# facebookresearch/lightplane

Hardware: AMD Instinct MI355X
Metric: Mrays/sec fwd+bwd, 64^3x16ch triplane @128 samples; peak bwd mem (MB) (higher is better)
Workload: dtype f32

## Files before the change

### lightplane_amd/csrc/lp_mfma_common.h

```cpp
#pragma once
#include <stdlib.h>

#include "lp_device.h"
#include "lp_splat_walk.h"
#include "lp_host.h"
#include "lp_plane_range.h"

namespace lp {

typedef float f32x16 __attribute__((ext_vector_type(16)));

LP_DEV constexpr int featq(int q, int h) { return (q & 3) + 8 * (q >> 2) + 4 * h; }

#define LP_MFMA(a, b, c) __builtin_amdgcn_mfma_f32_32x32x2f32((a), (b), (c), 0, 0, 0)

LP_DEV int opaque_zero() {
  int z = 0;
  asm volatile("" : "+s"(z));
  return z;
}

constexpr int HID = 32;
constexpr int W_LD = 33;
constexpr int WAVES = 4;
// ... 18 lines not shown
};

struct Lds {
  static constexpr int WT1 = 0;
  static constexpr int WT2 = WT1 + 32 * W_LD;
  static constexpr int WO1 = WT2 + 32 * W_LD;
  static constexpr int WC1 = WO1 + 32 * W_LD;
  static constexpr int BIAS = WC1 + 32 * W_LD;
  static constexpr int WO2 = BIAS + 4 * 32;
  static constexpr int WC2 = WO2 + 32;
  static constexpr int HB = WC2 + 32 * 4;
  static constexpr int INF = HB + 8;
  static constexpr int FWD_END = INF + MAX_INF;
};

LP_DEV f32x16 load_bias(const float* lds, int which, int h, int zo) {
  const float4* b = reinterpret_cast<const float4*>(lds + Lds::BIAS + which * 32 + 4 * h + zo);
  f32x16 acc;
#pragma unroll
  for (int j = 0; j < 4; ++j) {
    const float4 v = b[2 * j];
    acc[4 * j + 0] = v.x; acc[4 * j + 1] = v.y; acc[4 * j + 2] = v.z; acc[4 * j + 3] = v.w;
  }
  return acc;
}

LP_DEV int wave_min_i(int v) {
#pragma unroll
  for (int m = 32; m >= 1; m >>= 1) { const int o = __shfl_xor(v, m); v = o < v ? o : v; }
  return __builtin_amdgcn_readfirstlane(v);
}
struct WaveRanges {
  unsigned lo3, hi3;
  static constexpr unsigned G = 0x20080200u;
  LP_DEV unsigned mask(int s) const {
    s = __builtin_amdgcn_readfirstlane(s);
    const unsigned sss = (unsigned)(s < 511 ? s : 511) * 0x00100401u;
    return ((sss | G) - lo3) & ((hi3 | G) - sss) & G;
  }
  static constexpr unsigned bit(int g) { return 0x200u << (10 * g); }
};
constexpr int RANGE_MAX_S = 511;
LP_DEV WaveRanges wave_ranges_full() { return WaveRanges{0u, 0x1ff7fdffu}; }
template <int GM>
LP_DEV WaveRanges wave_plane_ranges(const LpRendererArgs& a, const Ray& ray, bool valid, bool plain) {
  WaveRanges w = wave_ranges_full();
  if (GM == GM_GENERIC) return w;
  const int S = a.march.num_samples;
  if (!plain || S > RANGE_MAX_S || __ballot(!valid) != 0) return w;
  const LpGrid* g = a.grid.grids;
  const int W = g[0].W, H = g[0].H, D = (GM == GM_TRIPLANE) ? g[1].D : g[0].D;
  const AxisSpans ax = ray_axis_spans(ray.ox, ray.oy, ray.oz, ray.dx, ray.dy, ray.dz, ray.near_t, ray.far_t, S, W, H, D);
#pragma unroll
  for (int p = 0; p < (GM == GM_TRIPLANE ? 3 : 1); ++p) {
    const SampleSpan sp = (GM == GM_TRIPLANE) ? plane_span(ax, p, S) : voxel_span(ax, S);
    const int lo = wave_min_i(sp.lo), hi = -wave_min_i(-sp.hi);
    if (p == 0) w.lo3 = w.hi3 = 0u;
    w.lo3 |= (unsigned)(hi < lo ? 511 : lo) << (10 * p);
    w.hi3 |= (unsigned)(hi < lo ? 0 : hi) << (10 * p);
  }
  if (GM == GM_VOXEL) {
    w.lo3 *= 0x00100401u;
    w.hi3 *= 0x00100401u;
  }
  w.lo3 = (unsigned)__builtin_amdgcn_readfirstlane((int)w.lo3);
  w.hi3 = (unsigned)__builtin_amdgcn_readfirstlane((int)w.hi3);
  return w;
}

template <int C>
LP_DEV void gather_tap(const float* data, int row, float w, int h, float (&x0)[C / 2]) {
  const float4* src = reinterpret_cast<const float4*>(data + (int64_t)(row < 0 ? 0 : row) * C + 4 * h);
#pragma unroll
  for (int j = 0; j < C / 8; ++j) {
    const float4 v = src[2 * j];
    x0[4 * j + 0] = fmaf(w, v.x, x0[4 * j + 0]);
    x0[4 * j + 1] = fmaf(w, v.y, x0[4 * j + 1]);
    x0[4 * j + 2] = fmaf(w, v.z, x0[4 * j + 2]);
    x0[4 * j + 3] = fmaf(w, v.w, x0[4 * j + 3]);
  }
}

template <int C>
LP_DEV void gather_taps4(const float* data, const int* row, const float* w, float keep, int h, float (&x0)[C / 2]) {
  float4 v[4][C / 8];
#pragma unroll
  for (int k = 0; k < 4; ++k) {
    const float4* src = reinterpret_cast<const float4*>(data + (int64_t)(row[k] < 0 ? 0 : row[k]) * C + 4 * h);
#pragma unroll
    for (int j = 0; j < C / 8; ++j) v[k][j] = src[2 * j];
  }
  __builtin_amdgcn_sched_barrier(0);
#pragma unroll
  for (int k = 0; k < 4; ++k) {
    const float wk = w[k] * keep;
#pragma unroll
    for (int j = 0; j < C / 8; ++j) {
      x0[4 * j + 0] = fmaf(wk, v[k][j].x, x0[4 * j + 0]);
      x0[4 * j + 1] = fmaf(wk, v[k][j].y, x0[4 * j + 1]);
      x0[4 * j + 2] = fmaf(wk, v[k][j].z, x0[4 * j + 2]);
// ... 498 lines not shown
```

### lightplane_amd/csrc/lp_plane_range.h

```cpp
#pragma once
#include <math.h>

#if defined(__HIPCC__)
#define LP_HD __host__ __device__ inline
#else
#define LP_HD inline
#endif

namespace lp {

struct SampleSpan {
  int lo, hi;
};

LP_HD SampleSpan span_full(int S) { return SampleSpan{0, S - 1}; }
LP_HD SampleSpan span_none(int S) { return SampleSpan{S, -1}; }
LP_HD SampleSpan span_meet(SampleSpan a, SampleSpan b, int S) {
  const SampleSpan m{a.lo > b.lo ? a.lo : b.lo, a.hi < b.hi ? a.hi : b.hi};
  return m.lo > m.hi ? span_none(S) : m;
}
LP_HD SampleSpan span_hull(SampleSpan a, SampleSpan b) {
  return SampleSpan{a.lo < b.lo ? a.lo : b.lo, a.hi > b.hi ? a.hi : b.hi};
}

LP_HD SampleSpan axis_sample_span(float o, float d, float near_t, float far_t, int S, int size) {
  if (S < 2) return span_full(S);
  const float L = 1.0f + 1.0f / (float)size;
  const float per = (float)(S - 1) / (far_t - near_t);
  const float inv = 1.0f / d;
  float s0 = ((-L - o) * inv - near_t) * per;
  float s1 = ((L - o) * inv - near_t) * per;
  if (s0 > s1) { const float t = s0; s0 = s1; s1 = t; }
  const float err = 1.9073486e-6f * fabsf(per) * ((L + fabsf(o)) * fabsf(inv) + fabsf(near_t) + fabsf(far_t));
  if (!(err < 0.5f)) return span_full(S);
  if (!(s0 <= (float)S && s1 >= -1.0f)) return span_none(S);
  const int lo = (int)floorf(fmaxf(s0, 0.0f)) - 1;
  const int hi = (int)ceilf(fminf(s1, (float)(S - 1))) + 1;
  return SampleSpan{lo < 0 ? 0 : lo, hi > S - 1 ? S - 1 : hi};
}

struct AxisSpans {
  SampleSpan x, y, z;
};
LP_HD AxisSpans ray_axis_spans(float ox, float oy, float oz, float dx, float dy, float dz, float near_t, float far_t, int S, int W,
                               int H, int D) {
  return AxisSpans{axis_sample_span(ox, dx, near_t, far_t, S, W), axis_sample_span(oy, dy, near_t, far_t, S, H),
                   axis_sample_span(oz, dz, near_t, far_t, S, D)};
}
LP_HD SampleSpan plane_span(const AxisSpans& a, int g, int S) {
  return g == 0 ? span_meet(a.x, a.y, S) : (g == 1 ? span_meet(a.x, a.z, S) : span_meet(a.y, a.z, S));
}
LP_HD SampleSpan voxel_span(const AxisSpans& a, int S) { return span_meet(span_meet(a.x, a.y, S), a.z, S); }

}
```

### lightplane_amd/csrc/lp_renderer_mfma.hip

```cpp
#include "lp_mfma_common.h"
#include "lp_bf3.h"

namespace lp {

template <int C, int GM, int OCC, int NC, bool SEGF = false>
__global__ void __launch_bounds__(256, OCC) renderer_fwd_bf3(const LpRendererArgs a, const MfmaParams mp) {
  extern __shared__ __attribute__((aligned(16))) float lds[];
  stage_weights_bf3<C>(a, mp, lds, false, 256);
  __syncthreads();
  const float* sm = lds - Lds::BIAS;
  const char* fimg = reinterpret_cast<const char*>(lds) + LdsBf3<C>::FWD_IMG;
  const int lane = threadIdx.x & 63, wave = threadIdx.x >> 6;
  const int h = lane >> 5, r = lane & 31;
  const int seg_len = LP_SEG_LEN * mp.seg_blocks;
  const int n_seg = SEGF ? (a.march.num_samples + seg_len - 1) / seg_len : 1;
  const int blk = SEGF ? (int)blockIdx.x / n_seg : (int)blockIdx.x;
  const int seg = SEGF ? (int)blockIdx.x - blk * n_seg : 0;
  const int64_t ray_id = ((int64_t)blk * WAVES + wave) * RAYS_PER_WAVE + r;
  const bool valid = ray_id < a.rays.n_rays;
  const int64_t rid = valid ? ray_id : 0;
  const Ray ray = load_ray(a.rays, rid);
  float cb[16];
  {
    float enc[16];
    load_encoding(a, rid, h, enc);
    color_prebias_bf3<C>(sm, fimg, lane, enc, cb);
  }
  const int s_tot = a.march.num_samples + a.march.num_samples_inf;
  const int n_ckpt = ckpt_count(a.march);
  const float delta0 = (a.march.num_samples > 1) ? (ray.far_t - ray.near_t) / (float)(a.march.num_samples - 1) : 1.0f;
  float nlt = 0.0f, nlt_lo = 0.0f, t_prev = 1.0f, len = 0.0f, depth_prev = 0.0f;
  int s_last = s_tot - 1;
  float facc[4] = {0.0f, 0.0f, 0.0f, 0.0f};
  Sample<C> nx;
  Act<C> t;
  const int s_lo = SEGF ? seg * seg_len : 0;
  const int s_hi = SEGF ? ((s_lo + seg_len < s_tot) ? s_lo + seg_len : s_tot) : s_tot;
  const bool plain_march = !SEGF && a.march.num_samples_inf == 0 && !a.march.contract_coords && !a.scaffold && !(a.noise_sigma > 0.0f);
  const WaveRanges rg = wave_plane_ranges<GM>(a, ray, valid, plain_march);
  if (SEGF && s_lo > 0) {
    sample_geometry<C>(a, sm, ray, s_lo - 1, nx);
    depth_prev = nx.depth;
  }
  for (int s = s_lo; s < s_hi; ++s) {
    fetch_sample<C, GM, true>(a, sm, ray, s, h, nx, rg.mask(s));
    const float depth = nx.depth, occ = nx.occ;
#pragma unroll
    for (int q = 0; q < C / 2; ++q) t.x0[q] = nx.x0[q];
    const int zo = opaque_zero();
    const Heads hd = decode_bf3<C, NC>(sm, fimg, lane, cb, t, zo);
    const float delta = (s == 0) ? delta0 : depth - depth_prev;
    depth_prev = depth;
    float raw = hd.raw_o;
    if (a.noise_sigma > 0.0f) raw = raw + sample_noise(rid, s, a.rays.n_rays, s_tot, a.noise_seed) * a.noise_sigma;
    const float opacity = a.gain * softplus_f(raw) * occ;
    nlt_add(nlt, nlt_lo, opacity * delta);
    if (!SEGF && a.neg_log_t_ckpt && valid && h == 0) {
      const int ck = ckpt_index(s, a.march);
      if (ck >= 0) *reinterpret_cast<float2*>(a.neg_log_t_ckpt + (ray_id * n_ckpt + ck) * 2) = make_float2(nlt, nlt_lo);
    }
    const float tr = __expf(-nlt);
    const float w = t_prev - tr;
    t_prev = tr;
    len = fmaf(w, depth, len);
#pragma unroll
    for (int c = 0; c < NC; ++c) facc[c] = fmaf(w, sigmoid_f(hd.raw_c[c]) * occ, facc[c]);
    if (a.seg_prefix && valid && h == 0 && (((s + 1) % LP_SEG_LEN) == 0 || s == a.march.num_samples - 1)) {
      float4* dst = reinterpret_cast<float4*>(a.seg_prefix + (ray_id * segment_count(a.march) + s / LP_SEG_LEN) * 8);
      dst[0] = make_float4(len, facc[0], facc[1], facc[2]);
      dst[1] = make_float4(NC == 4 ? facc[3] : 0.0f, nlt, nlt_lo, 0.0f);
    }
    if (a.stop_neg_log_t > 0.0f && __ballot(valid && nlt < a.stop_neg_log_t) == 0) {
      s_last = s;
      break;
    }
  }
  if (!SEGF && valid && h == 0) {
    write_ray_outputs(a, ray_id, len, nlt, facc);
    if (a.neg_log_t_ckpt)
      *reinterpret_cast<float2*>(a.neg_log_t_ckpt + (ray_id * n_ckpt + n_ckpt - 1) * 2) = make_float2((float)s_last, nlt_lo);
  }
}

// ... 300 lines not shown
```

### lightplane_amd/csrc/lp_renderer_mfma_bwd.h

```cpp
#pragma once
#include "lp_mfma_common.h"
#include <type_traits>

#include "lp_bf3.h"

namespace lp {

#ifdef LP_ASM_MARKS
#define LP_MARK(n) asm volatile("; LPMARK " n)
#else
#define LP_MARK(n)
#endif
typedef float f32x4 __attribute__((ext_vector_type(4)));
#define LP_MFMA16(a, b, c) __builtin_amdgcn_mfma_f32_16x16x4f32((a), (b), (c), 0, 0, 0)

constexpr int T_LD = 36;

LP_DEV constexpr int pi16(int m) { return m < 4 ? 2 * m : (m < 12 ? 2 * (m - 4) + 1 : 2 * (m - 8)); }

LP_DEV void lds_barrier() { asm volatile("s_waitcnt lgkmcnt(0)\n\ts_barrier" ::: "memory"); }

LP_DEV void tile_store_fm(float* tile, int r, int h, const float (&v)[16]) {
#pragma unroll
  for (int q = 0; q < 16; ++q) tile[featq(q, h) * T_LD + r] = v[q];
// ... 34 lines not shown
  const u32x2_t ua = __builtin_bit_cast(u32x2_t, a), ub = __builtin_bit_cast(u32x2_t, b);
  return (u32x4_t){ua.x, ua.y, ub.x, ub.y};
}
template <int STRIDE_BYTES>
LP_DEV f32x4 dw_quadrant_bf(const char* wave0b, int x_off, int y_off, int v0, int v1, f32x4 acc, f32x4& acc_db, unsigned onehot, bool do_db = true) {
  const u32x4_t oh = {onehot, onehot, onehot, onehot};
#pragma unroll 1
  for (int v = v0; v < v1; ++v) {
    const char* base = wave0b + v * STRIDE_BYTES;
    const u32x4_t b2 = limb_tile_operand(base + y_off + LT_LIMB);
    const u32x4_t a1 = limb_tile_operand(base + x_off);
    if (do_db) acc_db = LP_MFMA16B(oh, b2, acc_db);
    acc = LP_MFMA16B(a1, b2, acc);
    const u32x4_t b1 = limb_tile_operand(base + y_off);
    if (do_db) acc_db = LP_MFMA16B(oh, b1, acc_db);
    acc = LP_MFMA16B(a1, b1, acc);
    const u32x4_t a2 = limb_tile_operand(base + x_off + LT_LIMB);
    acc = LP_MFMA16B(a2, b1, acc);
  }
  return acc;
}

struct LdsB3 {
  static constexpr int XT = 0;
  static constexpr int YT = 32 * T_LD;
  static constexpr int TS = 2 * 32 * T_LD;
  static constexpr int PER_WAVE = TS + 5 * 32;
};
template <int C, int NW>
struct Bf3Lds {
  static constexpr int IMG_END = (NW == 8) ? LdsBf3<C>::BWD_END : LdsBf3Rm<C>::END;
  static constexpr int CB = IMG_END + NW * LdsB3::PER_WAVE * 4;
  static constexpr bool CB_LDS = (NW == 8) ? (C == 16) : (CB + NW * 64 * 16 * 4) * 2 <= 160 * 1024;
  static constexpr int TOTAL = CB + (CB_LDS ? NW * 64 * 16 * 4 : 0);
};

template <int C, int GM, bool PLAIN, int NC, int NW, bool SEG = false, bool DUMP = false, bool F32 = false>
__global__ void __launch_bounds__(64 * NW, NW == 8 ? 1 : 2) renderer_bwd_bf3(const LpRendererArgs a, const MfmaParams mp) {
  constexpr int DXL = F32 ? 3 : 2;
  constexpr bool DWB = !F32;
  using M = Lds;
  using L = LdsBf3<C>;
  using R = LdsBf3Rm<C>;
  using B = LdsB3;
  constexpr int WAVES3 = NW;
  extern __shared__ __attribute__((aligned(16))) float lds[];
  if (NW == 8) stage_weights_bf3<C>(a, mp, lds, true, 64 * NW);
  else stage_weights_rm<C>(a, mp, lds, 64 * NW);
  const float* const sm = lds - M::BIAS;
  const char* const fimg = reinterpret_cast<const char*>(lds) + L::FWD_IMG;
  const char* const bimg = reinterpret_cast<const char*>(lds) + L::BWD_IMG;
  const char* const rimg = reinterpret_cast<const char*>(lds);
  const int lane = threadIdx.x & 63;
  const int wave = __builtin_amdgcn_readfirstlane((int)(threadIdx.x >> 6));
  const int h = lane >> 5, r = lane & 31;
  float* const wave0 = reinterpret_cast<float*>(reinterpret_cast<char*>(lds) + Bf3Lds<C, NW>::IMG_END);
  float* const wv = wave0 + wave * B::PER_WAVE;
  float* const xt = wv + B::XT;
  float* const yt = wv + B::YT;
  float* const ts = wv + B::TS;

  constexpr bool seg_on = SEG;
  const int n_rec = seg_on ? segment_count(a.march) : 1;
  const int seg_len = LP_SEG_LEN * mp.seg_blocks;
  const int n_seg = seg_on ? (a.march.num_samples + seg_len - 1) / seg_len : 1;
  const int blk = seg_on ? (int)blockIdx.x / n_seg : (int)blockIdx.x;
  const int seg = seg_on ? (int)blockIdx.x - blk * n_seg : 0;
// ... 63 lines not shown
  auto rho = [](int k) { return (k & 0x15) | ((k & 2) << 2) | ((k & 8) >> 2); };
  char* const xrow = reinterpret_cast<char*>(wv) + B::XT * 4 + rm_off(rho(r), 4 * h);
  char* const yrow = xrow + (B::YT - B::XT) * 4;
  const int xq_off = B::XT * 4 + rm_off(rho(8 * ka + (m16 >> 2)), 4 * (m16 & 3)) + 32 * mi;
  const int yq_off = B::YT * 4 + rm_off(rho(8 * ka + (m16 >> 2)), 4 * (m16 & 3)) + 32 * ni;
  f32x4 dq_b = {0, 0, 0, 0};
  auto onehot = [&](int li) -> unsigned { return (lane & 15) == li ? 0x3F803F80u : 0u; };
  const int a_off_t1 = (C == 16) ? B::XT + pi16(m16) * T_LD + 8 * ka : a_off;
  const int t1_v0 = (C == 16) ? 2 * (wave >> 1) : v0, t1_v1 = (C == 16) ? 2 * (wave >> 1) + 2 : v0 + 4;
  f32x4 dq_t1 = {0, 0, 0, 0}, dq_t2 = {0, 0, 0, 0}, dq_o1 = {0, 0, 0, 0}, dq_c1 = {0, 0, 0, 0};
  float db_t1 = 0.0f, db_t2 = 0.0f, db_o1 = 0.0f, db_c1 = 0.0f;
  float dwo2 = 0.0f, dwc2[4] = {0.0f, 0.0f, 0.0f, 0.0f};
  float dbo2 = 0.0f, dbc2[4] = {0.0f, 0.0f, 0.0f, 0.0f};
  const bool gg = a.grad_grid_list[0] != nullptr;

  float nlt = a.neg_log_t[rid];
  float suffix = 0.0f, p_next = 0.0f;
  if (seg_on) {
    const float4* pj = reinterpret_cast<const float4*>(a.seg_prefix + (rid * n_rec + s_begin / LP_SEG_LEN) * 8);
    const float4* pt = reinterpret_cast<const float4*>(a.seg_prefix + (rid * n_rec + n_rec - 1) * 8);
    const float4 j0 = pj[0], j1 = pj[1], t0 = pt[0];
    nlt = j1.y;
    nlt_lo = j1.z;
    if (seg < n_seg - 1) {
      float rest = g_len * (t0.x - j0.x);
      rest = fmaf(gfeat[0], t0.y - j0.y, rest);
      rest = fmaf(gfeat[1], t0.z - j0.z, rest);
      rest = fmaf(gfeat[2], t0.w - j0.w, rest);
      if (NC == 4) rest = fmaf(gfeat[3], pt[1].x - j1.x, rest);
      suffix = -rest;
    }
  }
  const WaveRanges rg = wave_plane_ranges<GM>(a, ray, valid, PLAIN && !SEG);
  Sample<C> nx;
  fetch_sample<C, GM, false, PLAIN>(a, sm, ray, s_begin, h, nx);
  for (int s = s_begin; s >= s_lo; --s) {
    const bool on = PLAIN || s <= s_last_w;
    const unsigned pm = rg.mask(s);
    const bool ggs = gg && pm != 0u;
    const float depth = nx.depth, occ = nx.occ, x = nx.x, y = nx.y, z = nx.z;
    float x0[C / 2];
#pragma unroll
    for (int q = 0; q < C / 2; ++q) x0[q] = nx.x0[q];
    const int zo = opaque_zero();
    const float* ldz = sm + zo;
    auto Af = [&](auto layer) {
      constexpr int l = decltype(layer)::value;
      if constexpr (NW == 8) return ASlots{fimg + zo, l == 0 ? L::CH_T1 : l == 1 ? L::CH_T2 : l == 2 ? L::CH_O1 : L::CH_C1};
      else return AColsFwd{rimg + zo + (l == 0 ? R::L_T1 : l == 1 ? R::L_T2 : l == 2 ? R::L_O1 : R::L_C1), l == 0 ? R::ST_T1 : R::ST_32};
    };
    auto Ab = [&](auto layer) {
      constexpr int l = decltype(layer)::value;
      if constexpr (NW == 8) return ASlots{bimg + zo, l == 0 ? L::CB_T1 : l == 1 ? L::CB_T2 : l == 2 ? L::CB_O1 : L::CB_C1};
      else return ARowsBwd{rimg + zo + (l == 0 ? R::L_T1 : l == 1 ? R::L_T2 : l == 2 ? R::L_O1 : R::L_C1), l == 0 ? R::ST_T1 : R::ST_32,
                           l == 0 ? C - 1 : 31};
    };
    using I0 = std::integral_constant<int, 0>; using I1 = std::integral_constant<int, 1>;
    using I2 = std::integral_constant<int, 2>; using I3 = std::integral_constant<int, 3>;

    LP_MARK("fwd");
    float h1[16];
    float e[16];
    unsigned ho_mask = 0, hc_mask = 0;
    Heads hd;
    {
      f32x16 acc;
      {
        acc = layer_bf3v<C / 16>(Af(I0{}), lane, x0, load_bias(sm, 0, h, zo));
#pragma unroll
        for (int q = 0; q < 16; ++q) h1[q] = relu_f(acc[q]);
      }
      acc = layer_bf3v<2>(Af(I1{}), lane, h1, load_bias(sm, 1, h, zo));
#pragma unroll
      for (int q = 0; q < 16; ++q) {
        e[q] = relu_f(acc[q]);
      }
      float ho[16], hc[16];
      {
        f32x16 acc_o = load_bias(sm, 2, h, zo), acc_c;
        if (CBL) {
#pragma unroll
          for (int i = 0; i < 4; ++i) {
            const float4 v = *reinterpret_cast<const float4*>(cbt + zo + ((i + cb_rot) & 3) * 4);
            acc_c[4 * i] = v.x; acc_c[4 * i + 1] = v.y; acc_c[4 * i + 2] = v.z; acc_c[4 * i + 3] = v.w;
          }
        } else {
#pragma unroll
          for (int q = 0; q < 16; ++q) acc_c[q] = cb[q];
        }
        layer2_bf3v<2>(Af(I2{}), Af(I3{}), lane, e, acc_o, acc_c);
#pragma unroll
        for (int q = 0; q < 16; ++q) {
          ho[q] = relu_f(acc_o[q]);
          hc[q] = relu_f(acc_c[q]);
        }
      }
      hd = heads_forward<NC>(sm, h, ho, hc, zo);
#pragma unroll
      for (int q = 0; q < 16; ++q) {
        ho_mask = mask_bit(ho_mask, ho[q], q);
        hc_mask = mask_bit(hc_mask, hc[q], q);
      }
      if constexpr (DUMP) {
        unsigned m1 = 0, m2 = 0, mo = 0, mc = 0;
#pragma unroll
        for (int q = 0; q < 16; ++q) {
          const unsigned bit = 1u << featq(q, h);
          m1 |= (h1[q] > 0.0f) ? bit : 0u;
          m2 |= (e[q] > 0.0f) ? bit : 0u;
          mo |= ((ho_mask >> q) & 1u) ? bit : 0u;
          mc |= ((hc_mask >> q) & 1u) ? bit : 0u;
        }
        m1 |= __shfl_xor(m1, 32); m2 |= __shfl_xor(m2, 32); mo |= __shfl_xor(mo, 32); mc |= __shfl_xor(mc, 32);
        if (valid && h == 0) {
          uint32_t* d = mp.relu_dump + (rid * s_tot + s) * 5;
          d[0] = m1; d[1] = m2; d[2] = mo; d[3] = mc; d[4] = on ? 1u : 2u;
        }
      }
      LP_SCHED_FENCE();
      if (want_params) {
        tile_store_fm(xt, r, h, ho);
        tile_store_fm(yt, r, h, hc);
      }
      LP_SCHED_FENCE();
    }

    LP_MARK("compositing");
    const float depth_prev =
        PLAIN ? ray.near_t + lin01((s > 0) ? s - 1 : 0, a.march.num_samples) * (ray.far_t - ray.near_t)
              : sample_depth_tab((s > 0) ? s - 1 : 0, a.march, ray.near_t, ray.far_t, sm + M::INF);
    const float delta = (s == 0) ? delta0 : depth - depth_prev;
    float raw = hd.raw_o;
    if (!PLAIN && a.noise_sigma > 0.0f)
      raw = raw + sample_noise(rid, s, a.rays.n_rays, s_tot, a.noise_seed) * a.noise_sigma;
    const float opacity = a.gain * softplus_f(raw) * occ;
    if (on && a.neg_log_t_ckpt) {
      const int ck = PLAIN ? ((((s + 1) % LP_NLT_CKPT) == 0 || s == s_tot - 1) ? s / LP_NLT_CKPT : -1)
                           : ckpt_index(s, a.march);
      if (ck >= 0) {
        const float2 c2 = *reinterpret_cast<const float2*>(a.neg_log_t_ckpt + (rid * n_ckpt + ck) * 2);
        nlt = c2.x;
        nlt_lo = c2.y;
      }
    }
    const float t_i = __expf(-nlt);
    nlt_add(nlt, nlt_lo, on ? -(opacity * delta) : 0.0f);
    if (!(nlt > 0.0f)) { nlt = 0.0f; nlt_lo = 0.0f; }
    const float t_im1 = __expf(-nlt);
    const float w = t_im1 - t_i;
    float sg[4];
    float p_i = g_len * depth;
#pragma unroll
    for (int c = 0; c < 4; ++c) {
      sg[c] = (c < NC) ? sigmoid_f(hd.raw_c[c]) : 0.0f;
      if (c < NC) p_i = fmaf(gfeat[c], sg[c] * occ, p_i);
    }
    suffix = on ? fmaf(t_i, p_i - p_next, suffix) : suffix;
    p_next = on ? p_i : p_next;
    const float d_a = suffix + g_nlt;
    const bool contrib = valid && on;
    const float dro = contrib ? d_a * delta * a.gain * occ * d_softplus_f(raw) : 0.0f;
    float drc[4];
#pragma unroll
    for (int c = 0; c < 4; ++c) drc[c] = (c < NC && contrib) ? w * gfeat[c] * occ * sg[c] * (1.0f - sg[c]) : 0.0f;

    LP_MARK("heads_bwd");
    float dhc[16];
    {
      const float* wc2 = sm + M::WC2 + 16 * h + opaque_zero();
#pragma unroll
      for (int j = 0; j < 4; ++j) {
#pragma unroll
        for (int i = 0; i < 4; ++i) {
          const int q = 4 * j + i;
          const float4 wc = *reinterpret_cast<const float4*>(wc2 + (8 * j + i) * 4);
          float v = drc[0] * wc.x;
          v = fmaf(drc[1], wc.y, v);
          v = fmaf(drc[2], wc.z, v);
          if (NC > 3) v = fmaf(drc[3], wc.w, v);
          dhc[q] = mask_apply(hc_mask, q, v);
        }
        LP_SCHED_FENCE();
      }
    }
    if (h == 0) {
      dbo2 += dro;
#pragma unroll
      for (int c = 0; c < NC; ++c) dbc2[c] += drc[c];
    }
    if (want_params) {
      if (h == 0) {
        ts[r] = dro;
#pragma unroll
        for (int c = 0; c < NC; ++c) ts[(1 + c) * 32 + r] = drc[c];
      }
      const float* xf = xt + r * T_LD + 16 * h;
      const float* yf = yt + r * T_LD + 16 * h;
      const float* tf = ts + 16 * h;
#pragma unroll
      for (int i = 0; i < 4; ++i) {
        const float4 hov = *reinterpret_cast<const float4*>(xf + 4 * i);
        const float4 hcv = *reinterpret_cast<const float4*>(yf + 4 * i);
        const float4 d0 = *reinterpret_cast<const float4*>(tf + 4 * i);
        dwo2 = fmaf(hov.x, d0.x, dwo2); dwo2 = fmaf(hov.y, d0.y, dwo2);
        dwo2 = fmaf(hov.z, d0.z, dwo2); dwo2 = fmaf(hov.w, d0.w, dwo2);
#pragma unroll
        for (int c = 0; c < NC; ++c) {
          const float4 dc = *reinterpret_cast<const float4*>(tf + (1 + c) * 32 + 4 * i);
          dwc2[c] = fmaf(hcv.x, dc.x, dwc2[c]); dwc2[c] = fmaf(hcv.y, dc.y, dwc2[c]);
          dwc2[c] = fmaf(hcv.z, dc.z, dwc2[c]); dwc2[c] = fmaf(hcv.w, dc.w, dwc2[c]);
        }
        LP_SCHED_FENCE();
      }
    }
    LP_SCHED_FENCE();

    LP_MARK("c1");
#ifndef LP_NO_PRIO
    __builtin_amdgcn_s_setprio(1);
#endif
    f32x16 acc = (f32x16){0};
    {
      if constexpr (DWB) {
        if (want_params) limb_tile_store<2>(xrow, e);
        acc = layer_dxv<2, DXL>(Ab(I3{}), lane, dhc, acc, want_params ? yrow : nullptr);
      } else {
        if (want_params) {
          tile_store_fm(xt, r, h, e);
          tile_store_fm(yt, r, h, dhc);
        }
        acc = layer_dxv<2, DXL>(Ab(I3{}), lane, dhc, acc);
      }
#pragma unroll
      for (int q = 0; q < 16; ++q) dsum[q] += dhc[q];
      if (want_params) {
        lds_barrier();
        if constexpr (DWB) dq_c1 = dw_quadrant_bf<B::PER_WAVE * 4>(reinterpret_cast<const char*>(wave0), xq_off, yq_off, v0, v0 + 4, dq_c1, dq_b, onehot(0));
        else dq_c1 = dw_quadrant<B::PER_WAVE>(wave0, a_off, b_off, v0, v0 + 4, dq_c1, db_c1);
        lds_barrier();
      }
    }
    LP_SCHED_FENCE();
    LP_MARK("o1");
    {
      float dho[16];
#pragma unroll
      for (int j = 0; j < 4; ++j) {
        const float4 wo = *reinterpret_cast<const float4*>(ldz + M::WO2 + 8 * j + 4 * h);
        dho[4 * j + 0] = mask_apply(ho_mask, 4 * j + 0, dro * wo.x);
        dho[4 * j + 1] = mask_apply(ho_mask, 4 * j + 1, dro * wo.y);
        dho[4 * j + 2] = mask_apply(ho_mask, 4 * j + 2, dro * wo.z);
        dho[4 * j + 3] = mask_apply(ho_mask, 4 * j + 3, dro * wo.w);
      }
      if constexpr (DWB) {
        acc = layer_dxv<2, DXL>(Ab(I2{}), lane, dho, acc, want_params ? yrow : nullptr);
      } else {
        if (want_params) tile_store_fm(yt, r, h, dho);
        acc = layer_dxv<2, DXL>(Ab(I2{}), lane, dho, acc);
      }
      if (want_params) {
        lds_barrier();
        if constexpr (DWB) dq_o1 = dw_quadrant_bf<B::PER_WAVE * 4>(reinterpret_cast<const char*>(wave0), xq_off, yq_off, v0, v0 + 4, dq_o1, dq_b, onehot(1));
        else dq_o1 = dw_quadrant<B::PER_WAVE>(wave0, a_off, b_off, v0, v0 + 4, dq_o1, db_o1);
        lds_barrier();
      }
    }
    float de[16];
#pragma unroll
    for (int q = 0; q < 16; ++q) de[q] = (e[q] > 0.0f) ? acc[q] : 0.0f;
    LP_SCHED_FENCE();
    LP_MARK("t2");
    float dh1[16];
    {
      if constexpr (DWB) {
        if (want_params) limb_tile_store<2>(xrow, h1);
        acc = layer_dxv<2, DXL>(Ab(I1{}), lane, de, (f32x16){0}, want_params ? yrow : nullptr);
      } else {
        if (want_params) {
          tile_store_fm(xt, r, h, h1);
          tile_store_fm(yt, r, h, de);
        }
        acc = layer_dxv<2, DXL>(Ab(I1{}), lane, de, (f32x16){0});
      }
      if (want_params) {
        lds_barrier();
        if constexpr (DWB) dq_t2 = dw_quadrant_bf<B::PER_WAVE * 4>(reinterpret_cast<const char*>(wave0), xq_off, yq_off, v0, v0 + 4, dq_t2, dq_b, onehot(2));
        else dq_t2 = dw_quadrant<B::PER_WAVE>(wave0, a_off, b_off, v0, v0 + 4, dq_t2, db_t2);
      }
#pragma unroll
      for (int q = 0; q < 16; ++q) dh1[q] = (h1[q] > 0.0f) ? acc[q] : 0.0f;
      if (want_params) lds_barrier();
    }
    LP_SCHED_FENCE();
    LP_MARK("t1");
    {
      if constexpr (DWB) {
        if (want_params) limb_tile_store<C / 16>(xrow, x0);
        if (ggs) {
          acc = layer_dxv<2, DXL>(Ab(I0{}), lane, dh1, (f32x16){0}, want_params ? yrow : nullptr);
        } else if (want_params) {
          limb_tile_store<2>(yrow, dh1);
        }
      } else {
        if (want_params) {
#pragma unroll
          for (int q = 0; q < C / 2; ++q) xt[featq(q, h) * T_LD + r] = x0[q];
          tile_store_fm(yt, r, h, dh1);
        }
        if (ggs) {
          acc = layer_dxv<2, DXL>(Ab(I0{}), lane, dh1, (f32x16){0});
        }
      }
      if (want_params) {
        lds_barrier();
        if constexpr (DWB) dq_t1 = dw_quadrant_bf<B::PER_WAVE * 4>(reinterpret_cast<const char*>(wave0), (C == 16) ? xq_off - 32 * mi : xq_off, yq_off, t1_v0, t1_v1, dq_t1, dq_b, onehot(3));
        else dq_t1 = dw_quadrant<B::PER_WAVE>(wave0, a_off_t1, b_off, t1_v0, t1_v1, dq_t1, db_t1);
        lds_barrier();
      }
    }
    if (ggs) {
#pragma unroll
      for (int q = 0; q < C / 2; ++q) xt[featq(q, h) * DX_LD + r] = acc[q];
    }
    LP_SCHED_FENCE();
    LP_MARK("fetch");
    __builtin_amdgcn_s_setprio(0);
    const bool live = valid && on && !(a.march.mask_out_of_bounds && !point_in_bounds(x, y, z));
    if (s > s_lo) fetch_sample<C, GM, true, PLAIN>(a, sm, ray, s - 1, h, nx, rg.mask(s - 1));
    LP_SCHED_FENCE();
    LP_MARK("scatter");
    if (ggs) {
      if constexpr (GM == GM_TRIPLANE) {
        scatter_triplane<C>(a.grad_grid_list, a.grid, ray.b, x, y, z, live, lane, xt, yt, pm);
      } else {
        const int ng = (GM == GM_VOXEL) ? 1 : a.grid.n_grids;
#pragma unroll 1
        for (int g = 0; g < ng; ++g)
          scatter_grid<C, GM>(a.grad_grid_list[g], a.grid.grids[g], ray.b, x, y, z, live, lane, xt, yt);
      }
    }
  }

  LP_MARK("epilogue");
  {
    f32x16 acc;
    if constexpr (NW == 8) acc = layer_bf3v<2>(ASlots{bimg, L::CB_C1}, lane, dsum, (f32x16){0});
    else acc = layer_bf3v<2>(ARowsBwd{rimg + R::L_C1, R::ST_32, 31}, lane, dsum, (f32x16){0});
    if (valid && a.grad_encoding && !seg_on) {
      float4* dst = reinterpret_cast<float4*>(a.grad_encoding + ray_id * HID + 4 * h);
#pragma unroll
      for (int j = 0; j < 4; ++j) dst[2 * j] = make_float4(acc[4 * j], acc[4 * j + 1], acc[4 * j + 2], acc[4 * j + 3]);
    } else if (valid && a.grad_encoding) {
      float* dst = a.grad_encoding + ray_id * HID + 4 * h;
#pragma unroll
      for (int j = 0; j < 4; ++j)
#pragma unroll
        for (int i = 0; i < 4; ++i) atomic_add_f32(dst + 8 * j + i, acc[4 * j + i]);
    }
  }
  if (want_params) {
    {
// ... 134 lines not shown
```

Measured before the change: 30.94.

## Skip MLP recompute and backprop for samples outside all planes via constant-feature shortcut

Samples where every plane mask is empty see zero features, so their MLP outputs are the same constant. The forward pass and backward pass now compute this zero-feature MLP once per wave or workgroup and reuse it for those samples. In the backward pass, gradients from skipped samples are accumulated and pushed through the MLP once in a single deferred extra iteration. This is meant to remove per-sample MLP work in empty regions, at the cost of extra LDS, a workgroup-wide range exchange with barriers, and more complex control flow.

Result: no change. 31.30 (median of 6 runs) (+1.1%).

```diff
diff --git a/lightplane_amd/csrc/lp_mfma_common.h b/lightplane_amd/csrc/lp_mfma_common.h
--- a/lightplane_amd/csrc/lp_mfma_common.h
+++ b/lightplane_amd/csrc/lp_mfma_common.h
@@ -74,16 +74,21 @@
 }
 struct WaveRanges {
   unsigned lo3, hi3;
-  static constexpr unsigned G = 0x20080200u;
+  static constexpr unsigned G = RANGE3_GUARD;
   LP_DEV unsigned mask(int s) const {
     s = __builtin_amdgcn_readfirstlane(s);
-    const unsigned sss = (unsigned)(s < 511 ? s : 511) * 0x00100401u;
-    return ((sss | G) - lo3) & ((hi3 | G) - sss) & G;
+    return range3_mask(lo3, hi3, s);
   }
   static constexpr unsigned bit(int g) { return 0x200u << (10 * g); }
+  LP_DEV bool any_empty(int s0, int s1) const {
+    if (lo3 == RANGE3_FULL_LO && hi3 == RANGE3_FULL_HI) return false;
+    bool any = false;
+    for (int s = s0; s <= s1; ++s) any = any || mask(s) == 0u;
+    return any;
+  }
 };
-constexpr int RANGE_MAX_S = 511;
-LP_DEV WaveRanges wave_ranges_full() { return WaveRanges{0u, 0x1ff7fdffu}; }
+constexpr int RANGE_MAX_S = RANGE3_MAX_S;
+LP_DEV WaveRanges wave_ranges_full() { return WaveRanges{RANGE3_FULL_LO, RANGE3_FULL_HI}; }
 template <int GM>
 LP_DEV WaveRanges wave_plane_ranges(const LpRendererArgs& a, const Ray& ray, bool valid, bool plain) {
   WaveRanges w = wave_ranges_full();
@@ -93,21 +98,34 @@
   const LpGrid* g = a.grid.grids;
   const int W = g[0].W, H = g[0].H, D = (GM == GM_TRIPLANE) ? g[1].D : g[0].D;
   const AxisSpans ax = ray_axis_spans(ray.ox, ray.oy, ray.oz, ray.dx, ray.dy, ray.dz, ray.near_t, ray.far_t, S, W, H, D);
+  w.lo3 = w.hi3 = 0u;
 #pragma unroll
   for (int p = 0; p < (GM == GM_TRIPLANE ? 3 : 1); ++p) {
     const SampleSpan sp = (GM == GM_TRIPLANE) ? plane_span(ax, p, S) : voxel_span(ax, S);
-    const int lo = wave_min_i(sp.lo), hi = -wave_min_i(-sp.hi);
-    if (p == 0) w.lo3 = w.hi3 = 0u;
-    w.lo3 |= (unsigned)(hi < lo ? 511 : lo) << (10 * p);
-    w.hi3 |= (unsigned)(hi < lo ? 0 : hi) << (10 * p);
+    range3_set(w.lo3, w.hi3, p, SampleSpan{wave_min_i(sp.lo), -wave_min_i(-sp.hi)});
   }
   if (GM == GM_VOXEL) {
-    w.lo3 *= 0x00100401u;
-    w.hi3 *= 0x00100401u;
+    w.lo3 *= RANGE3_ONES;
+    w.hi3 *= RANGE3_ONES;
   }
   w.lo3 = (unsigned)__builtin_amdgcn_readfirstlane((int)w.lo3);
   w.hi3 = (unsigned)__builtin_amdgcn_readfirstlane((int)w.hi3);
   return w;
+}
+template <int NW>
+LP_DEV WaveRanges workgroup_ranges(const WaveRanges& w, unsigned* xch, int wave, int lane) {
+  if (lane == 0) {
+    xch[2 * wave] = w.lo3;
+    xch[2 * wave + 1] = w.hi3;
+  }
+  __syncthreads();
+  WaveRanges g = w;
+#pragma unroll
+  for (int v = 0; v < NW; ++v) range3_hull(g.lo3, g.hi3, xch[2 * v], xch[2 * v + 1]);
+  __syncthreads();
+  g.lo3 = (unsigned)__builtin_amdgcn_readfirstlane((int)g.lo3);
+  g.hi3 = (unsigned)__builtin_amdgcn_readfirstlane((int)g.hi3);
+  return g;
 }
 
 template <int C>
diff --git a/lightplane_amd/csrc/lp_plane_range.h b/lightplane_amd/csrc/lp_plane_range.h
--- a/lightplane_amd/csrc/lp_plane_range.h
+++ b/lightplane_amd/csrc/lp_plane_range.h
@@ -52,4 +52,28 @@
 }
 LP_HD SampleSpan voxel_span(const AxisSpans& a, int S) { return span_meet(span_meet(a.x, a.y, S), a.z, S); }
 
+constexpr int RANGE3_MAX_S = 511;
+constexpr unsigned RANGE3_GUARD = 0x20080200u;
+constexpr unsigned RANGE3_ONES = 0x00100401u;
+constexpr unsigned RANGE3_FULL_LO = 0u, RANGE3_FULL_HI = 0x1ff7fdffu;
+LP_HD void range3_set(unsigned& lo3, unsigned& hi3, int p, SampleSpan sp) {
+  lo3 |= (unsigned)(sp.hi < sp.lo ? 511 : sp.lo) << (10 * p);
+  hi3 |= (unsigned)(sp.hi < sp.lo ? 0 : sp.hi) << (10 * p);
 }
+LP_HD unsigned range3_mask(unsigned lo3, unsigned hi3, int s) {
+  const unsigned sss = (unsigned)(s < 511 ? s : 511) * RANGE3_ONES;
+  return ((sss | RANGE3_GUARD) - lo3) & ((hi3 | RANGE3_GUARD) - sss) & RANGE3_GUARD;
+}
+LP_HD void range3_hull(unsigned& lo3, unsigned& hi3, unsigned l, unsigned h) {
+  unsigned lo = 0u, hi = 0u;
+  for (int p = 0; p < 3; ++p) {
+    const unsigned a = (lo3 >> (10 * p)) & 511u, b = (l >> (10 * p)) & 511u;
+    const unsigned c = (hi3 >> (10 * p)) & 511u, d = (h >> (10 * p)) & 511u;
+    lo |= (a < b ? a : b) << (10 * p);
+    hi |= (c > d ? c : d) << (10 * p);
+  }
+  lo3 = lo;
+  hi3 = hi;
+}
+
+}
diff --git a/lightplane_amd/csrc/lp_renderer_mfma.hip b/lightplane_amd/csrc/lp_renderer_mfma.hip
--- a/lightplane_amd/csrc/lp_renderer_mfma.hip
+++ b/lightplane_amd/csrc/lp_renderer_mfma.hip
@@ -42,13 +42,26 @@
     sample_geometry<C>(a, sm, ray, s_lo - 1, nx);
     depth_prev = nx.depth;
   }
+  Heads hd0 = {};
+  if (!SEGF && GM != GM_GENERIC && rg.any_empty(s_lo, s_hi - 1)) {
+#pragma unroll
+    for (int q = 0; q < C / 2; ++q) t.x0[q] = 0.0f;
+    hd0 = decode_bf3<C, NC>(sm, fimg, lane, cb, t, opaque_zero());
+    hd0.raw_o = __builtin_bit_cast(float, __builtin_amdgcn_readfirstlane(__builtin_bit_cast(int, hd0.raw_o)));
+  }
   for (int s = s_lo; s < s_hi; ++s) {
-    fetch_sample<C, GM, true>(a, sm, ray, s, h, nx, rg.mask(s));
+    const unsigned pm = rg.mask(s);
+    Heads hd;
+    if (!SEGF && GM != GM_GENERIC && pm == 0u) {
+      sample_geometry<C>(a, sm, ray, s, nx);
+      hd = hd0;
+    } else {
+      fetch_sample<C, GM, true>(a, sm, ray, s, h, nx, pm);
+#pragma unroll
+      for (int q = 0; q < C / 2; ++q) t.x0[q] = nx.x0[q];
+      hd = decode_bf3<C, NC>(sm, fimg, lane, cb, t, opaque_zero());
+    }
     const float depth = nx.depth, occ = nx.occ;
-#pragma unroll
-    for (int q = 0; q < C / 2; ++q) t.x0[q] = nx.x0[q];
-    const int zo = opaque_zero();
-    const Heads hd = decode_bf3<C, NC>(sm, fimg, lane, cb, t, zo);
     const float delta = (s == 0) ? delta0 : depth - depth_prev;
     depth_prev = depth;
     float raw = hd.raw_o;
diff --git a/lightplane_amd/csrc/lp_renderer_mfma_bwd.h b/lightplane_amd/csrc/lp_renderer_mfma_bwd.h
--- a/lightplane_amd/csrc/lp_renderer_mfma_bwd.h
+++ b/lightplane_amd/csrc/lp_renderer_mfma_bwd.h
@@ -90,7 +90,10 @@
   static constexpr int IMG_END = (NW == 8) ? LdsBf3<C>::BWD_END : LdsBf3Rm<C>::END;
   static constexpr int CB = IMG_END + NW * LdsB3::PER_WAVE * 4;
   static constexpr bool CB_LDS = (NW == 8) ? (C == 16) : (CB + NW * 64 * 16 * 4) * 2 <= 160 * 1024;
-  static constexpr int TOTAL = CB + (CB_LDS ? NW * 64 * 16 * 4 : 0);
+  static constexpr int KZ = CB + (CB_LDS ? NW * 64 * 16 * 4 : 0);
+  static constexpr int KZ_ROOM = ((NW == 8 ? 160 : 80) * 1024 - KZ) / (NW * 32 * 4);
+  static constexpr int KZ_N = KZ_ROOM < 0 ? 0 : (KZ_ROOM > 4 ? 4 : KZ_ROOM);
+  static constexpr int TOTAL = KZ + KZ_N * NW * 32 * 4;
 };
 
 template <int C, int GM, bool PLAIN, int NC, int NW, bool SEG = false, bool DUMP = false, bool F32 = false>
@@ -220,100 +223,62 @@
     }
   }
   const WaveRanges rg = wave_plane_ranges<GM>(a, ray, valid, PLAIN && !SEG);
-  Sample<C> nx;
-  fetch_sample<C, GM, false, PLAIN>(a, sm, ray, s_begin, h, nx);
-  for (int s = s_begin; s >= s_lo; --s) {
+  auto Af = [&](auto layer, int zo) {
+    constexpr int l = decltype(layer)::value;
+    if constexpr (NW == 8) return ASlots{fimg + zo, l == 0 ? L::CH_T1 : l == 1 ? L::CH_T2 : l == 2 ? L::CH_O1 : L::CH_C1};
+    else return AColsFwd{rimg + zo + (l == 0 ? R::L_T1 : l == 1 ? R::L_T2 : l == 2 ? R::L_O1 : R::L_C1), l == 0 ? R::ST_T1 : R::ST_32};
+  };
+  auto Ab = [&](auto layer, int zo) {
+    constexpr int l = decltype(layer)::value;
+    if constexpr (NW == 8) return ASlots{bimg + zo, l == 0 ? L::CB_T1 : l == 1 ? L::CB_T2 : l == 2 ? L::CB_O1 : L::CB_C1};
+    else return ARowsBwd{rimg + zo + (l == 0 ? R::L_T1 : l == 1 ? R::L_T2 : l == 2 ? R::L_O1 : R::L_C1), l == 0 ? R::ST_T1 : R::ST_32,
+                         l == 0 ? C - 1 : 31};
+  };
+  using I0 = std::integral_constant<int, 0>; using I1 = std::integral_constant<int, 1>;
+  using I2 = std::integral_constant<int, 2>; using I3 = std::integral_constant<int, 3>;
+  auto recompute = [&](const float (&x0)[C / 2], float (&h1)[16], float (&e)[16], float (&ho)[16], float (&hc)[16], int zo, int ln) -> Heads {
+    const int hh = ln >> 5;
+    f32x16 acc = layer_bf3v<C / 16>(Af(I0{}, zo), ln, x0, load_bias(sm, 0, hh, zo));
+#pragma unroll
+    for (int q = 0; q < 16; ++q) h1[q] = relu_f(acc[q]);
+    acc = layer_bf3v<2>(Af(I1{}, zo), ln, h1, load_bias(sm, 1, hh, zo));
+#pragma unroll
+    for (int q = 0; q < 16; ++q) e[q] = relu_f(acc[q]);
+    f32x16 acc_o = load_bias(sm, 2, hh, zo), acc_c;
+    if (CBL) {
+#pragma unroll
+      for (int i = 0; i < 4; ++i) {
+        const float4 v = *reinterpret_cast<const float4*>(cbt + zo + ((i + cb_rot) & 3) * 4);
+        acc_c[4 * i] = v.x; acc_c[4 * i + 1] = v.y; acc_c[4 * i + 2] = v.z; acc_c[4 * i + 3] = v.w;
+      }
+    } else {
+#pragma unroll
+      for (int q = 0; q < 16; ++q) acc_c[q] = cb[q];
+    }
+    layer2_bf3v<2>(Af(I2{}, zo), Af(I3{}, zo), ln, e, acc_o, acc_c);
+#pragma unroll
+    for (int q = 0; q < 16; ++q) {
+      ho[q] = relu_f(acc_o[q]);
+      hc[q] = relu_f(acc_c[q]);
+    }
+    return heads_forward<NC>(sm, hh, ho, hc, zo);
+  };
+  auto relu_words = [&](const float (&h1)[16], const float (&e)[16], const float (&ho)[16], const float (&hc)[16], unsigned (&m)[4]) {
+    m[0] = m[1] = m[2] = m[3] = 0u;
+#pragma unroll
+    for (int q = 0; q < 16; ++q) {
+      const unsigned bit = 1u << featq(q, h);
+      m[0] |= (h1[q] > 0.0f) ? bit : 0u;
+      m[1] |= (e[q] > 0.0f) ? bit : 0u;
+      m[2] |= (ho[q] > 0.0f) ? bit : 0u;
+      m[3] |= (hc[q] > 0.0f) ? bit : 0u;
+    }
+#pragma unroll
+    for (int i = 0; i < 4; ++i) m[i] |= __shfl_xor(m[i], 32);
+  };
+
+  auto composite = [&](int s, float depth, float occ, const Heads& hd, float& dro, float (&drc)[4]) {
     const bool on = PLAIN || s <= s_last_w;
-    const unsigned pm = rg.mask(s);
-    const bool ggs = gg && pm != 0u;
-    const float depth = nx.depth, occ = nx.occ, x = nx.x, y = nx.y, z = nx.z;
-    float x0[C / 2];
-#pragma unroll
-    for (int q = 0; q < C / 2; ++q) x0[q] = nx.x0[q];
-    const int zo = opaque_zero();
-    const float* ldz = sm + zo;
-    auto Af = [&](auto layer) {
-      constexpr int l = decltype(layer)::value;
-      if constexpr (NW == 8) return ASlots{fimg + zo, l == 0 ? L::CH_T1 : l == 1 ? L::CH_T2 : l == 2 ? L::CH_O1 : L::CH_C1};
-      else return AColsFwd{rimg + zo + (l == 0 ? R::L_T1 : l == 1 ? R::L_T2 : l == 2 ? R::L_O1 : R::L_C1), l == 0 ? R::ST_T1 : R::ST_32};
-    };
-    auto Ab = [&](auto layer) {
-      constexpr int l = decltype(layer)::value;
-      if constexpr (NW == 8) return ASlots{bimg + zo, l == 0 ? L::CB_T1 : l == 1 ? L::CB_T2 : l == 2 ? L::CB_O1 : L::CB_C1};
-      else return ARowsBwd{rimg + zo + (l == 0 ? R::L_T1 : l == 1 ? R::L_T2 : l == 2 ? R::L_O1 : R::L_C1), l == 0 ? R::ST_T1 : R::ST_32,
-                           l == 0 ? C - 1 : 31};
-    };
-    using I0 = std::integral_constant<int, 0>; using I1 = std::integral_constant<int, 1>;
-    using I2 = std::integral_constant<int, 2>; using I3 = std::integral_constant<int, 3>;
-
-    LP_MARK("fwd");
-    float h1[16];
-    float e[16];
-    unsigned ho_mask = 0, hc_mask = 0;
-    Heads hd;
-    {
-      f32x16 acc;
-      {
-        acc = layer_bf3v<C / 16>(Af(I0{}), lane, x0, load_bias(sm, 0, h, zo));
-#pragma unroll
-        for (int q = 0; q < 16; ++q) h1[q] = relu_f(acc[q]);
-      }
-      acc = layer_bf3v<2>(Af(I1{}), lane, h1, load_bias(sm, 1, h, zo));
-#pragma unroll
-      for (int q = 0; q < 16; ++q) {
-        e[q] = relu_f(acc[q]);
-      }
-      float ho[16], hc[16];
-      {
-        f32x16 acc_o = load_bias(sm, 2, h, zo), acc_c;
-        if (CBL) {
-#pragma unroll
-          for (int i = 0; i < 4; ++i) {
-            const float4 v = *reinterpret_cast<const float4*>(cbt + zo + ((i + cb_rot) & 3) * 4);
-            acc_c[4 * i] = v.x; acc_c[4 * i + 1] = v.y; acc_c[4 * i + 2] = v.z; acc_c[4 * i + 3] = v.w;
-          }
-        } else {
-#pragma unroll
-          for (int q = 0; q < 16; ++q) acc_c[q] = cb[q];
-        }
-        layer2_bf3v<2>(Af(I2{}), Af(I3{}), lane, e, acc_o, acc_c);
-#pragma unroll
-        for (int q = 0; q < 16; ++q) {
-          ho[q] = relu_f(acc_o[q]);
-          hc[q] = relu_f(acc_c[q]);
-        }
-      }
-      hd = heads_forward<NC>(sm, h, ho, hc, zo);
-#pragma unroll
-      for (int q = 0; q < 16; ++q) {
-        ho_mask = mask_bit(ho_mask, ho[q], q);
-        hc_mask = mask_bit(hc_mask, hc[q], q);
-      }
-      if constexpr (DUMP) {
-        unsigned m1 = 0, m2 = 0, mo = 0, mc = 0;
-#pragma unroll
-        for (int q = 0; q < 16; ++q) {
-          const unsigned bit = 1u << featq(q, h);
-          m1 |= (h1[q] > 0.0f) ? bit : 0u;
-          m2 |= (e[q] > 0.0f) ? bit : 0u;
-          mo |= ((ho_mask >> q) & 1u) ? bit : 0u;
-          mc |= ((hc_mask >> q) & 1u) ? bit : 0u;
-        }
-        m1 |= __shfl_xor(m1, 32); m2 |= __shfl_xor(m2, 32); mo |= __shfl_xor(mo, 32); mc |= __shfl_xor(mc, 32);
-        if (valid && h == 0) {
-          uint32_t* d = mp.relu_dump + (rid * s_tot + s) * 5;
-          d[0] = m1; d[1] = m2; d[2] = mo; d[3] = mc; d[4] = on ? 1u : 2u;
-        }
-      }
-      LP_SCHED_FENCE();
-      if (want_params) {
-        tile_store_fm(xt, r, h, ho);
-        tile_store_fm(yt, r, h, hc);
-      }
-      LP_SCHED_FENCE();
-    }
-
-    LP_MARK("compositing");
     const float depth_prev =
         PLAIN ? ray.near_t + lin01((s > 0) ? s - 1 : 0, a.march.num_samples) * (ray.far_t - ray.near_t)
               : sample_depth_tab((s > 0) ? s - 1 : 0, a.march, ray.near_t, ray.far_t, sm + M::INF);
@@ -326,7 +291,10 @@
       const int ck = PLAIN ? ((((s + 1) % LP_NLT_CKPT) == 0 || s == s_tot - 1) ? s / LP_NLT_CKPT : -1)
                            : ckpt_index(s, a.march);
       if (ck >= 0) {
-        const float2 c2 = *reinterpret_cast<const float2*>(a.neg_log_t_ckpt + (rid * n_ckpt + ck) * 2);
+        int ln = lane;
+        asm volatile("" : "+v"(ln));
+        const int64_t rid2 = valid ? ((int64_t)blk * WAVES3 + wave) * RAYS_PER_WAVE + (ln & 31) : 0;
+        const float2 c2 = *reinterpret_cast<const float2*>(a.neg_log_t_ckpt + (rid2 * n_ckpt + ck) * 2);
         nlt = c2.x;
         nlt_lo = c2.y;
       }
@@ -347,11 +315,125 @@
     p_next = on ? p_i : p_next;
     const float d_a = suffix + g_nlt;
     const bool contrib = valid && on;
-    const float dro = contrib ? d_a * delta * a.gain * occ * d_softplus_f(raw) : 0.0f;
-    float drc[4];
+    dro = contrib ? d_a * delta * a.gain * occ * d_softplus_f(raw) : 0.0f;
 #pragma unroll
     for (int c = 0; c < 4; ++c) drc[c] = (c < NC && contrib) ? w * gfeat[c] * occ * sg[c] * (1.0f - sg[c]) : 0.0f;
-
+  };
+
+  constexpr bool SKIP = PLAIN && !SEG && GM != GM_GENERIC;
+  WaveRanges sk = rg;
+  bool any_skip = false;
+  constexpr int KZL = Bf3Lds<C, NW>::KZ_N < NC ? Bf3Lds<C, NW>::KZ_N : NC;
+  float* const kzw = reinterpret_cast<float*>(reinterpret_cast<char*>(lds) + Bf3Lds<C, NW>::KZ) + wave * (Bf3Lds<C, NW>::KZ_N * 32);
+  float kz_o = 0.0f;
+  float kz_c[NC > KZL ? NC - KZL : 1];
+  auto skipped_sum = [&](float v) { const float o = __shfl_xor(v, 32); return h ? v : o; };
+  unsigned dump0[4] = {0u, 0u, 0u, 0u};
+#pragma unroll
+  for (int i = 0; i < (NC > KZL ? NC - KZL : 1); ++i) kz_c[i] = 0.0f;
+  if constexpr (SKIP) {
+    sk = workgroup_ranges<NW>(rg, reinterpret_cast<unsigned*>(wave0), wave, lane);
+    any_skip = sk.any_empty(s_lo, s_begin);
+    if (any_skip) {
+      float x0[C / 2], h1[16], e[16], ho[16], hc[16];
+#pragma unroll
+      for (int q = 0; q < C / 2; ++q) x0[q] = 0.0f;
+      int ln = lane;
+      asm volatile("" : "+v"(ln));
+      const Heads hz = recompute(x0, h1, e, ho, hc, opaque_zero(), ln);
+      kz_o = __builtin_bit_cast(float, __builtin_amdgcn_readfirstlane(__builtin_bit_cast(int, hz.raw_o)));
+#pragma unroll
+      for (int c = 0; c < NC; ++c) {
+        if (c < KZL) kzw[(c < KZL ? c : 0) * 32 + r] = hz.raw_c[c];
+        else kz_c[c < KZL ? 0 : c - KZL] = hz.raw_c[c];
+      }
+      if constexpr (DUMP) relu_words(h1, e, ho, hc, dump0);
+    }
+  }
+  const int s_end = s_lo - (any_skip ? 1 : 0);
+  Sample<C> nx;
+  fetch_sample<C, GM, false, PLAIN>(a, sm, ray, s_begin, h, nx);
+  for (int s = s_begin; s >= s_end; --s) {
+    const bool deferred = SKIP && s < s_lo;
+    const bool on = PLAIN || s <= s_last_w;
+    const bool skip = SKIP && any_skip && !deferred && sk.mask(s) == 0u;
+    const unsigned pm = deferred ? 0u : rg.mask(s);
+    const bool ggs = gg && pm != 0u;
+    const float depth = nx.depth, occ = nx.occ, x = nx.x, y = nx.y, z = nx.z;
+    float x0[C / 2];
+#pragma unroll
+    for (int q = 0; q < C / 2; ++q) x0[q] = nx.x0[q];
+    const int zo = opaque_zero();
+    const float* ldz = sm + zo;
+
+    LP_MARK("fwd");
+    float h1[16];
+    float e[16];
+    unsigned ho_mask = 0, hc_mask = 0;
+    Heads hd;
+    if (skip) {
+      int ln = lane;
+      asm volatile("" : "+v"(ln));
+      const float* const kzl = kzw + (ln & 31);
+      hd.raw_o = kz_o;
+#pragma unroll
+      for (int c = 0; c < 4; ++c)
+        hd.raw_c[c] = (c >= NC) ? 0.0f : (c < KZL) ? kzl[(c < KZL ? c : 0) * 32] : kz_c[(c < KZL || c >= NC) ? 0 : c - KZL];
+      if constexpr (DUMP) {
+        if (valid && h == 0) {
+          uint32_t* d = mp.relu_dump + (rid * s_tot + s) * 5;
+          d[0] = dump0[0]; d[1] = dump0[1]; d[2] = dump0[2]; d[3] = dump0[3]; d[4] = 1u;
+        }
+      }
+    } else {
+      float ho[16], hc[16];
+      hd = recompute(x0, h1, e, ho, hc, zo, lane);
+#pragma unroll
+      for (int q = 0; q < 16; ++q) {
+        ho_mask = mask_bit(ho_mask, ho[q], q);
+        hc_mask = mask_bit(hc_mask, hc[q], q);
+      }
+      if constexpr (DUMP) {
+        unsigned m1 = 0, m2 = 0, mo = 0, mc = 0;
+#pragma unroll
+        for (int q = 0; q < 16; ++q) {
+          const unsigned bit = 1u << featq(q, h);
+          m1 |= (h1[q] > 0.0f) ? bit : 0u;
+          m2 |= (e[q] > 0.0f) ? bit : 0u;
+          mo |= ((ho_mask >> q) & 1u) ? bit : 0u;
+          mc |= ((hc_mask >> q) & 1u) ? bit : 0u;
+        }
+        m1 |= __shfl_xor(m1, 32); m2 |= __shfl_xor(m2, 32); mo |= __shfl_xor(mo, 32); mc |= __shfl_xor(mc, 32);
+        if (valid && h == 0 && !deferred) {
+          uint32_t* d = mp.relu_dump + (rid * s_tot + s) * 5;
+          d[0] = m1; d[1] = m2; d[2] = mo; d[3] = mc; d[4] = on ? 1u : 2u;
+        }
+      }
+      LP_SCHED_FENCE();
+      if (want_params) {
+        tile_store_fm(xt, r, h, ho);
+        tile_store_fm(yt, r, h, hc);
+      }
+      LP_SCHED_FENCE();
+    }
+
+    LP_MARK("compositing");
+    float dro, drc[4];
+    if (deferred) {
+      dro = skipped_sum(dbo2);
+#pragma unroll
+      for (int c = 0; c < 4; ++c) drc[c] = (c < NC) ? skipped_sum(dbc2[c < NC ? c : 0]) : 0.0f;
+    } else {
+      composite(s, depth, occ, hd, dro, drc);
+    }
+
+    if (skip) {
+      if (h == 1) {
+        dbo2 += dro;
+#pragma unroll
+        for (int c = 0; c < NC; ++c) dbc2[c] += drc[c];
+      }
+    } else {
     LP_MARK("heads_bwd");
     float dhc[16];
     {
@@ -411,13 +493,13 @@
     {
       if constexpr (DWB) {
         if (want_params) limb_tile_store<2>(xrow, e);
-        acc = layer_dxv<2, DXL>(Ab(I3{}), lane, dhc, acc, want_params ? yrow : nullptr);
+        acc = layer_dxv<2, DXL>(Ab(I3{}, zo), lane, dhc, acc, want_params ? yrow : nullptr);
       } else {
         if (want_params) {
           tile_store_fm(xt, r, h, e);
           tile_store_fm(yt, r, h, dhc);
         }
-        acc = layer_dxv<2, DXL>(Ab(I3{}), lane, dhc, acc);
+        acc = layer_dxv<2, DXL>(Ab(I3{}, zo), lane, dhc, acc);
       }
 #pragma unroll
       for (int q = 0; q < 16; ++q) dsum[q] += dhc[q];
@@ -441,10 +523,10 @@
         dho[4 * j + 3] = mask_apply(ho_mask, 4 * j + 3, dro * wo.w);
       }
       if constexpr (DWB) {
-        acc = layer_dxv<2, DXL>(Ab(I2{}), lane, dho, acc, want_params ? yrow : nullptr);
+        acc = layer_dxv<2, DXL>(Ab(I2{}, zo), lane, dho, acc, want_params ? yrow : nullptr);
       } else {
         if (want_params) tile_store_fm(yt, r, h, dho);
-        acc = layer_dxv<2, DXL>(Ab(I2{}), lane, dho, acc);
+        acc = layer_dxv<2, DXL>(Ab(I2{}, zo), lane, dho, acc);
       }
       if (want_params) {
         lds_barrier();
@@ -462,13 +544,13 @@
     {
       if constexpr (DWB) {
         if (want_params) limb_tile_store<2>(xrow, h1);
-        acc = layer_dxv<2, DXL>(Ab(I1{}), lane, de, (f32x16){0}, want_params ? yrow : nullptr);
+        acc = layer_dxv<2, DXL>(Ab(I1{}, zo), lane, de, (f32x16){0}, want_params ? yrow : nullptr);
       } else {
         if (want_params) {
           tile_store_fm(xt, r, h, h1);
           tile_store_fm(yt, r, h, de);
         }
-        acc = layer_dxv<2, DXL>(Ab(I1{}), lane, de, (f32x16){0});
+        acc = layer_dxv<2, DXL>(Ab(I1{}, zo), lane, de, (f32x16){0});
       }
       if (want_params) {
         lds_barrier();
@@ -485,7 +567,7 @@
       if constexpr (DWB) {
         if (want_params) limb_tile_store<C / 16>(xrow, x0);
         if (ggs) {
-          acc = layer_dxv<2, DXL>(Ab(I0{}), lane, dh1, (f32x16){0}, want_params ? yrow : nullptr);
+          acc = layer_dxv<2, DXL>(Ab(I0{}, zo), lane, dh1, (f32x16){0}, want_params ? yrow : nullptr);
         } else if (want_params) {
           limb_tile_store<2>(yrow, dh1);
         }
@@ -496,7 +578,7 @@
           tile_store_fm(yt, r, h, dh1);
         }
         if (ggs) {
-          acc = layer_dxv<2, DXL>(Ab(I0{}), lane, dh1, (f32x16){0});
+          acc = layer_dxv<2, DXL>(Ab(I0{}, zo), lane, dh1, (f32x16){0});
         }
       }
       if (want_params) {
@@ -509,12 +591,18 @@
     if (ggs) {
 #pragma unroll
       for (int q = 0; q < C / 2; ++q) xt[featq(q, h) * DX_LD + r] = acc[q];
+    }
     }
     LP_SCHED_FENCE();
     LP_MARK("fetch");
     __builtin_amdgcn_s_setprio(0);
     const bool live = valid && on && !(a.march.mask_out_of_bounds && !point_in_bounds(x, y, z));
-    if (s > s_lo) fetch_sample<C, GM, true, PLAIN>(a, sm, ray, s - 1, h, nx, rg.mask(s - 1));
+    if (s > s_lo) {
+      fetch_sample<C, GM, true, PLAIN>(a, sm, ray, s - 1, h, nx, rg.mask(s - 1));
+    } else if (SKIP && any_skip) {
+#pragma unroll
+      for (int q = 0; q < C / 2; ++q) nx.x0[q] = 0.0f;
+    }
     LP_SCHED_FENCE();
     LP_MARK("scatter");
     if (ggs) {
```
